# Monokaix/etcd

Hardware: AMD Instinct MI355X
Metric: quorum group-evals/sec at 1/2/4/8 MI355X; % HBM peak; speedup vs Go host (higher is better)
Workload: dtype u64; 1 GPU; config2_n5: 64M groups x 5-voter MajorityConfig CommittedIndex+VoteResult (TallyVotes counts into the stats); groups_per_gpu=67108864, global_groups=67108864, voters=5

## Files before the change

### etcd_amd/csrc/qe_api.hip

```cpp
#include <stdio.h>
#include <string.h>

#include "qe_dispatch.hpp"
#include "qe_conf.hpp"
#include "qe_collect.hpp"
#include "qe_tick.hpp"
#include "qe_follow.hpp"
#include "qe_vote.hpp"
#include "qe_snap.hpp"
#include "qe_outbox.hpp"
#include "qe_inbox.hpp"
#include "qe_replies.hpp"

namespace qe {

int g_blocks_per_cu = 0;
int g_nontemporal = 3;
int g_tiles_per_wave = -1;
int g_cv_kernel = -1;
int g_repl_kernel = -1;

static thread_local char g_errbuf[256];

void set_error(const char *msg) { snprintf(g_errbuf, sizeof(g_errbuf), "%s", msg); }

int hip_status(hipError_t e) {
  if (e == hipSuccess) return QE_OK;
  snprintf(g_errbuf, sizeof(g_errbuf), "HIP error %d: %s", static_cast<int>(e),
           hipGetErrorString(e));
  return QE_EHIP;
}

static inline bool al(const void *p, size_t a) {
  return (reinterpret_cast<uintptr_t>(p) % a) == 0;
}

static unsigned simple_grid(uint64_t G) {
  const uint64_t cap = static_cast<uint64_t>(num_cus()) * 8;
  const uint64_t need = (G + kBlock - 1) / kBlock;
  return static_cast<unsigned>(need < cap ? (need ? need : 1) : cap);
}

__global__ __launch_bounds__(kBlock) void k_apply_acks(uint64_t G, uint32_t S, uint64_t stride,
                                                       uint64_t *match, uint64_t *next,
                                                       uint64_t n, const uint64_t *group,
                                                       const int8_t *slot,
                                                       const uint64_t *index,
                                                       uint8_t *touched) {
  for (uint64_t i = static_cast<uint64_t>(blockIdx.x) * kBlock + threadIdx.x; i < n;
       i += static_cast<uint64_t>(gridDim.x) * kBlock) {
    const uint64_t g = group[i];
    const int s = slot[i];
    if (g >= G || s < 0 || s >= static_cast<int>(S)) continue;
    const uint64_t x = index[i];
    const uint64_t off = static_cast<uint64_t>(s) * stride + g;
    atomicMax(reinterpret_cast<unsigned long long *>(match + off),
              static_cast<unsigned long long>(x));
    if (x != ~0ull)
      atomicMax(reinterpret_cast<unsigned long long *>(next + off),
                static_cast<unsigned long long>(x + 1));
    if (touched) touched[g] = 1;
  }
}

__global__ void k_stats_reduce(const uint64_t *stats, uint64_t *out) {
  const int c = threadIdx.x;
  if (c < QE_STATS_COUNTERS) {
    uint64_t s = 0;
    for (int k = 0; k < QE_STATS_SHARDS; k++) s += stats[k * QE_STATS_COUNTERS + c];
    out[c] = s;
  }
}


}

using namespace qe;

template <class A>
static void step_head(const qe_progress *p, uint64_t *stats, A &a) {
  a.G = p->num_groups;
  a.goff = p->group_offset;
  a.stride = p->stride;
  a.R = p->log_runs;
  a.stats = stats;
}

extern "C" {

int qe_abi_version(void) { return QE_ABI_VERSION; }

const char *qe_strerror(int status) {
  switch (status) {
    case QE_OK: return "ok";
    case QE_EINVAL: return "invalid argument";
    case QE_ERANGE: return "out of range";
    case QE_EHIP: return g_errbuf[0] ? g_errbuf : "HIP error";
    case QE_ECOMM: return g_errbuf[0] ? g_errbuf : "RCCL error";
    default: return "unknown status";
  }
}

size_t qe_mask_bytes(uint32_t num_slots) {
  if (num_slots == 0 || num_slots > QE_MAX_SLOTS) return 0;
  return num_slots <= 8 ? 1 : 2;
}

int qe_tune(const char *key, int value) {
  if (!key) return QE_EINVAL;
  if (!strcmp(key, "blocks_per_cu")) {
    if (value < 0 || value > 32) return QE_ERANGE;
    g_blocks_per_cu = value;
    return QE_OK;
  }
  if (!strcmp(key, "tiles_per_wave")) {
    if (value < -1 || value > 4096) return QE_ERANGE;
    g_tiles_per_wave = value;
    return QE_OK;
  }
  if (!strcmp(key, "cv_kernel")) {
    if (value < -1 || value > 1) return QE_ERANGE;
    g_cv_kernel = value;
    return QE_OK;
  }
  if (!strcmp(key, "repl_kernel")) {
    if (value < -1 || value > 1) return QE_ERANGE;
    g_repl_kernel = value;
    return QE_OK;
  }
  if (!strcmp(key, "nontemporal")) {
    if (value < 0 || value > 3) return QE_ERANGE;
    g_nontemporal = value;
    return QE_OK;
  }
  return QE_EINVAL;
}

static int check_groups(const qe_groups *g) {
  if (!g) return QE_EINVAL;
  if (g->num_slots == 0 || g->num_slots > QE_MAX_SLOTS) return QE_EINVAL;
  if (g->reserved != 0) return QE_EINVAL;
  if (g->num_groups && g->stride < g->num_groups) return QE_EINVAL;
  if (g->out_mask && !g->inc_mask) return QE_EINVAL;
  return QE_OK;
}

int qe_commit_vote(const qe_groups *g, const qe_outputs *out, void *stream) {
  int rc = check_groups(g);
  if (rc) return rc;
  if (!out) return QE_EINVAL;
  if (g->num_groups == 0) return QE_OK;
  if (!g->match) return QE_EINVAL;
  CVArgs a{};
  a.G = g->num_groups;
  a.goff = g->group_offset;
  a.stride = g->stride;
  a.match = g->match;
  a.inc = g->inc_mask;
  a.out = g->out_mask;
  a.learner = g->learner_mask;
  a.voted = g->voted;
  a.granted = g->granted;
  a.commit = out->commit;
  a.vote = out->vote;
  a.gcount = out->granted_count;
  a.rcount = out->rejected_count;
  a.stats = out->stats;
  const int mode = g->out_mask ? 2 : (g->inc_mask ? 1 : 0);
  const size_t mb = qe_mask_bytes(g->num_slots);
  bool vec = al(g->match, 16) && (g->stride % 2 == 0) && al(out->commit, 16);
  const void *masks[] = {g->inc_mask, g->out_mask, g->learner_mask, g->voted, g->granted};
  for (const void *m : masks) vec = vec && al(m, 2 * mb);
  const uint8_t *bytes[] = {out->vote, out->granted_count, out->rejected_count};
  for (const uint8_t *b : bytes) vec = vec && al(b, 2);
  return with_slots(g->num_slots, [&](auto s) {
    return dispatch_cv<s()>(a, mode, vec, static_cast<hipStream_t>(stream));
  });
}

int qe_committed_index(const qe_groups *g, uint64_t *commit, void *stream) {
  if (!g || !commit) return QE_EINVAL;
  qe_groups gg = *g;
  gg.voted = nullptr;
  gg.granted = nullptr;
  qe_outputs o{};
  o.commit = commit;
  return qe_commit_vote(&gg, &o, stream);
}

int qe_vote_result(const qe_groups *g, uint8_t *vote, void *stream) {
  int rc = check_groups(g);
  if (rc) return rc;
  if (!vote) return QE_EINVAL;
  if (g->num_groups == 0) return QE_OK;
  const uint32_t full = (1u << g->num_slots) - 1u;
  hipStream_t st = static_cast<hipStream_t>(stream);
  const unsigned grid = simple_grid(g->num_groups);
  if (g->num_slots <= 8)
    hipLaunchKernelGGL(k_vote_result<uint8_t>, dim3(grid), dim3(kBlock), 0, st, g->num_groups,
                       full, g->inc_mask, g->out_mask, g->voted, g->granted, vote);
  else
    hipLaunchKernelGGL(k_vote_result<uint16_t>, dim3(grid), dim3(kBlock), 0, st,
                       g->num_groups, full, g->inc_mask, g->out_mask, g->voted, g->granted,
                       vote);
  return hip_status(hipGetLastError());
}

int qe_quorum_active(const qe_groups *g, const void *recent_active, uint8_t *active,
                     void *stream) {
  int rc = check_groups(g);
  if (rc) return rc;
  if (!recent_active || !active) return QE_EINVAL;
  if (g->num_groups == 0) return QE_OK;
  const uint32_t full = (1u << g->num_slots) - 1u;
  hipStream_t st = static_cast<hipStream_t>(stream);
  const unsigned grid = simple_grid(g->num_groups);
  if (g->num_slots <= 8)
    hipLaunchKernelGGL(k_quorum_active<uint8_t>, dim3(grid), dim3(kBlock), 0, st,
                       g->num_groups, full, g->inc_mask, g->out_mask, g->learner_mask,
                       recent_active, active);
  else
    hipLaunchKernelGGL(k_quorum_active<uint16_t>, dim3(grid), dim3(kBlock), 0, st,
                       g->num_groups, full, g->inc_mask, g->out_mask, g->learner_mask,
                       recent_active, active);
  return hip_status(hipGetLastError());
}

int qe_record_votes(uint64_t num_groups, uint32_t num_slots, void *voted, void *granted,
                    const void *resp_mask, const void *resp_value, void *stream) {
  if (num_slots == 0 || num_slots > QE_MAX_SLOTS) return QE_EINVAL;
  if (num_groups == 0) return QE_OK;
  if (!voted || !granted || !resp_mask || !resp_value) return QE_EINVAL;
  const uint32_t full = (1u << num_slots) - 1u;
  hipStream_t st = static_cast<hipStream_t>(stream);
  const unsigned grid = simple_grid(num_groups);
  if (num_slots <= 8)
    hipLaunchKernelGGL(k_record_votes<uint8_t>, dim3(grid), dim3(kBlock), 0, st, num_groups,
                       full, voted, granted, resp_mask, resp_value);
  else
    hipLaunchKernelGGL(k_record_votes<uint16_t>, dim3(grid), dim3(kBlock), 0, st, num_groups,
                       full, voted, granted, resp_mask, resp_value);
  return hip_status(hipGetLastError());
}

int qe_replication_round(const qe_repl_state *s, const qe_repl_msgs *m, uint64_t *stats,
                         void *stream) {
  if (!s || !m) return QE_EINVAL;
  if (s->num_slots == 0 || s->num_slots > QE_MAX_SLOTS || s->reserved) return QE_EINVAL;
  if (s->num_groups == 0) return QE_OK;
  if (s->stride < s->num_groups) return QE_EINVAL;
  if (!s->match || !s->next || !s->committed || !s->term_start || !s->last_index ||
      !m->resp_index)
    return QE_EINVAL;
  if (s->out_mask && !s->inc_mask) return QE_EINVAL;
  RArgs a{};
  a.G = s->num_groups;
  a.goff = s->group_offset;
  a.stride = s->stride;
  a.match = s->match;
  a.next = s->next;
  a.committed = s->committed;
  a.term_start = s->term_start;
  a.last_index = s->last_index;
  a.resp = m->resp_index;
  a.inc = s->inc_mask;
  a.out = s->out_mask;
  a.resp_mask = m->resp_mask;
  a.read_acks = m->read_acks;
  a.read_ok = m->read_ok;
  a.adv = m->commit_advanced;
  a.stats = stats;
  const size_t mb = qe_mask_bytes(s->num_slots);
  bool vec = (s->stride % 2 == 0);
  const void *p16[] = {s->match, s->next, s->committed, s->term_start, s->last_index,
                       m->resp_index};
// ... 940 lines not shown
```

### etcd_amd/csrc/qe_inst.hip

```cpp
#include "qe_dispatch.hpp"

#ifndef QE_S
#error "compile with -DQE_S=<slots>"
#endif
#ifndef QE_PAIRS
#define QE_PAIRS ((QE_S) <= 8 ? 2 : 1)
#endif

namespace qe {

namespace {
constexpr int S = QE_S;
using MT = std::conditional<(S <= 8), uint8_t, uint16_t>::type;

template <int MODE, bool VEC, bool NTL, bool NTS>
int launch_cv_k(const CVArgs &a, hipStream_t st) {
  constexpr int kPairs = QE_PAIRS;
  auto kern = k_commit_vote<S, MODE, MT, kPairs, VEC, NTL, NTS>;
  static int occ = occupancy(kern);
  const uint64_t npairs = (a.G + 1) / 2;
  const uint64_t tiles = (npairs + 64 * kPairs - 1) / (64 * kPairs);
  hipLaunchKernelGGL(kern, dim3(grid_for(tiles, occ, MODE == 2 ? 8 : 1)), dim3(kBlock), 0, st, a);
  return hip_status(hipGetLastError());
}

ChunkPlan stream_plan(uint64_t G) {
  return chunk_plan((G + 63) / 64, num_cus(), g_tiles_per_wave, QE_STREAM_TPW, false);
}

template <int MODE, bool NTL, bool NTS>
int launch_cv_stream(CVArgs a, hipStream_t st) {
  auto kern = k_cv_stream<S, MODE, MT, NTL, NTS>;
  const ChunkPlan plan = stream_plan(a.G);
  if (plan.status) return plan.status;
  a.chunk = plan.chunk;
  hipLaunchKernelGGL(kern, dim3(plan.blocks), dim3(kBlock), 0, st, a);
  return hip_status(hipGetLastError());
}

template <int MODE>
int launch_cv(const CVArgs &a, bool vec, hipStream_t st) {
  const int which = g_cv_kernel >= 0 ? g_cv_kernel : 1;
  if (which == 1)
    return with_nontemporal(g_nontemporal, [&](auto ntl, auto nts) {
      return launch_cv_stream<MODE, ntl(), nts()>(a, st);
    });
  if (!vec) return launch_cv_k<MODE, false, false, false>(a, st);
  return with_nontemporal(g_nontemporal, [&](auto ntl, auto nts) {
    return launch_cv_k<MODE, true, ntl(), nts()>(a, st);
  });
}
}

template <int N>
int dispatch_cv(const CVArgs &a, int mode, bool vec, hipStream_t st) {
  static_assert(N == S, "one slot count per object");
  switch (mode) {
    case 0: return launch_cv<0>(a, vec, st);
    case 1: return launch_cv<1>(a, vec, st);
    default: return launch_cv<2>(a, vec, st);
  }
}
template int dispatch_cv<S>(const CVArgs &, int, bool, hipStream_t);

template <bool J, bool M, bool V, bool NT>
static int launch_repl_k(const RArgs &a, hipStream_t st) {
  auto kern = k_replication<S, J, M, MT, V, NT>;
  static int occ = occupancy(kern);
  const uint64_t tiles = ((a.G + 1) / 2 + 63) / 64;
  hipLaunchKernelGGL(kern, dim3(grid_for(tiles, occ, 1)), dim3(kBlock), 0, st, a);
  return hip_status(hipGetLastError());
}

template <bool J, bool M, bool V>
static int launch_repl(const RArgs &a, hipStream_t st) {
  if (V && (g_nontemporal & 3) == 3) return launch_repl_k<J, M, V, true>(a, st);
  return launch_repl_k<J, M, V, false>(a, st);
}

template <bool M, bool J, bool NTL, bool NTS>
static int launch_repl_stream(RArgs a, hipStream_t st) {
  auto kern = k_repl_stream<S, M, J, MT, NTL, NTS>;
  const ChunkPlan plan = stream_plan(a.G);
  if (plan.status) return plan.status;
  a.chunk = plan.chunk;
  hipLaunchKernelGGL(kern, dim3(plan.blocks), dim3(kBlock), 0, st, a);
  return hip_status(hipGetLastError());
}

template <int N>
int dispatch_repl(const RArgs &a, bool masked, bool joint, bool vec, hipStream_t st) {
  static_assert(N == S, "one slot count per object");
  if (g_repl_kernel != 0)
    return with_quorum_form(masked, joint, [&](auto m, auto j) {
      return with_nontemporal(g_nontemporal, [&](auto ntl, auto nts) {
        return launch_repl_stream<m(), j(), ntl(), nts()>(a, st);
      });
    });
  if (vec)
    return with_quorum_form(masked, joint,
                            [&](auto m, auto j) { return launch_repl<j(), m(), true>(a, st); });
  return with_quorum_form(masked, joint,
                          [&](auto m, auto j) { return launch_repl<j(), m(), false>(a, st); });
}
template int dispatch_repl<S>(const RArgs &, bool, bool, bool, hipStream_t);

template <int OPT>
static int launch_elec(const EArgs &a, hipStream_t st) {
  auto kern = k_election<S, MT, OPT>;
  static int occ = occupancy(kern);
  const uint64_t waves = (a.G + 63) / 64;
  hipLaunchKernelGGL(kern, dim3(grid_for(waves, occ, 1)), dim3(kBlock), 0, st, a);
  return hip_status(hipGetLastError());
}

template <int N>
int dispatch_elec(const EArgs &a, hipStream_t st) {
  static_assert(N == S, "one slot count per object");
  const int opt = (a.flags & 3u) | (a.sresp ? 4 : 0) | (a.out ? 8 : 0);
  switch (opt) {
#define QE_E(o) \
  case o: return launch_elec<o>(a, st);
    QE_E(0) QE_E(1) QE_E(2) QE_E(3) QE_E(4) QE_E(5) QE_E(6) QE_E(7)
    QE_E(8) QE_E(9) QE_E(10) QE_E(11) QE_E(12) QE_E(13) QE_E(14)
#undef QE_E
    default: return launch_elec<15>(a, st);
  }
}
template int dispatch_elec<S>(const EArgs &, hipStream_t);

}
```

### etcd_amd/csrc/qe_kernels.hpp

```cpp
#pragma once
#if !defined(QE_VARIANT_BUILD) &&                                                      \
    (defined(QE_PSTEP_WAVES) || defined(QE_STREAM_TPW) || defined(QE_STREAM_WAVES) ||     \
     defined(QE_JOINT_MIN_WAVES) || defined(QE_LD_AUX) || defined(QE_ST_AUX) ||           \
     defined(QE_SEND_AUX) || defined(QE_SEND16_WAVES) || defined(QE_SWITCH16_WAVES) ||    \
     defined(QE_PROPOSE16_WAVES))
#error "A/B knob set in a product build: use scripts/build_variant*.sh (QE_VARIANT_BUILD)"
#endif
#include <hip/hip_runtime.h>

#include <stdint.h>
#include <stdio.h>
#include <string.h>

#include <type_traits>

#include "../../include/etcd_quorum.h"
#include "qe_device.hpp"
#include "qe_launch.hpp"

namespace qe {

typedef uint64_t u64x2 __attribute__((ext_vector_type(2)));

extern int g_blocks_per_cu;
extern int g_nontemporal;
extern int g_cv_kernel;
extern int g_repl_kernel;

inline int num_cus() {
  static int cached[64] = {0};
  int dev = 0;
  if (hipGetDevice(&dev) != hipSuccess || dev < 0 || dev >= 64) return 256;
  if (cached[dev] == 0) {
    int v = 0;
    if (hipDeviceGetAttribute(&v, hipDeviceAttributeMultiprocessorCount, dev) != hipSuccess ||
        v <= 0)
      v = 256;
    cached[dev] = v;
  }
  return cached[dev];
}

extern int g_tiles_per_wave;
inline unsigned grid_for(uint64_t work_waves, int occ, int auto_tpw = 0) {
  const uint64_t need = (work_waves + (kBlock / 64) - 1) / (kBlock / 64);
  const int tpw = g_tiles_per_wave >= 0 ? g_tiles_per_wave : auto_tpw;
  uint64_t g;
  if (tpw > 0) {
    g = (need + tpw - 1) / tpw;
  } else {
    int per_cu = occ > 0 ? occ : 4;
    if (g_blocks_per_cu > 0 && g_blocks_per_cu < per_cu) per_cu = g_blocks_per_cu;
    const uint64_t cap = static_cast<uint64_t>(num_cus()) * per_cu;
    g = need < cap ? need : cap;
  }
  if (g > 0x7FFFFFFFull) g = 0x7FFFFFFFull;
  return static_cast<unsigned>(g ? g : 1);
}

template <typename K>
inline int occupancy(K kernel) {
  int n = 0;
  if (hipOccupancyMaxActiveBlocksPerMultiprocessor(&n, kernel, kBlock, 0) != hipSuccess) n = 0;
  return n;
}

template <bool VEC, bool NT, bool GUARD = true>
__device__ __forceinline__ void ld_u64_pair(const uint64_t *p, uint64_t g0, uint64_t G,
                                            uint64_t &lo, uint64_t &hi) {
  if (VEC && (!GUARD || g0 + 1 < G)) {
    const u64x2 *q = reinterpret_cast<const u64x2 *>(p + g0);
    u64x2 x = NT ? __builtin_nontemporal_load(q) : *q;
    lo = x.x;
    hi = x.y;
  } else {
    lo = g0 < G ? p[g0] : 0;
    hi = g0 + 1 < G ? p[g0 + 1] : 0;
  }
}

template <bool VEC, bool NT = false, bool GUARD = true>
__device__ __forceinline__ void st_u64_pair(uint64_t *p, uint64_t g0, uint64_t G, uint64_t lo,
                                            uint64_t hi) {
  if (VEC && (!GUARD || g0 + 1 < G)) {
    u64x2 x;
    x.x = lo;
    x.y = hi;
    if (NT) __builtin_nontemporal_store(x, reinterpret_cast<u64x2 *>(p + g0));
    else *reinterpret_cast<u64x2 *>(p + g0) = x;
  } else {
    if (g0 < G) p[g0] = lo;
    if (g0 + 1 < G) p[g0 + 1] = hi;
  }
}

template <typename MT, bool VEC, bool GUARD = true>
__device__ __forceinline__ void ld_mask_pair(const void *p, uint64_t g0, uint64_t G,
                                             uint32_t &lo, uint32_t &hi) {
  const MT *m = static_cast<const MT *>(p);
  if (VEC && (!GUARD || g0 + 1 < G)) {
    if constexpr (sizeof(MT) == 1) {
      const uint32_t x = *reinterpret_cast<const uint16_t *>(m + g0);
      lo = x & 0xFFu;
      hi = x >> 8;
    } else {
      const uint32_t x = *reinterpret_cast<const uint32_t *>(m + g0);
      lo = x & 0xFFFFu;
      hi = x >> 16;
    }
  } else {
    lo = g0 < G ? m[g0] : 0u;
    hi = g0 + 1 < G ? m[g0 + 1] : 0u;
  }
}

template <typename MT, bool VEC, bool GUARD = true>
__device__ __forceinline__ void st_mask_pair(void *p, uint64_t g0, uint64_t G, uint32_t lo,
                                             uint32_t hi) {
  MT *m = static_cast<MT *>(p);
  if (VEC && (!GUARD || g0 + 1 < G)) {
    if constexpr (sizeof(MT) == 1) {
      *reinterpret_cast<uint16_t *>(m + g0) = static_cast<uint16_t>(lo | (hi << 8));
    } else {
      *reinterpret_cast<uint32_t *>(m + g0) = lo | (hi << 16);
    }
  } else {
    if (g0 < G) m[g0] = static_cast<MT>(lo);
    if (g0 + 1 < G) m[g0 + 1] = static_cast<MT>(hi);
  }
}

template <bool VEC, bool NT = false, bool GUARD = true>
__device__ __forceinline__ void st_u8_pair(uint8_t *p, uint64_t g0, uint64_t G, uint32_t lo,
                                           uint32_t hi) {
  if (VEC && (!GUARD || g0 + 1 < G)) {
    const uint16_t x = static_cast<uint16_t>(lo | (hi << 8));
    if (NT) __builtin_nontemporal_store(x, reinterpret_cast<uint16_t *>(p + g0));
    else *reinterpret_cast<uint16_t *>(p + g0) = x;
  } else {
    if (g0 < G) p[g0] = static_cast<uint8_t>(lo);
    if (g0 + 1 < G) p[g0 + 1] = static_cast<uint8_t>(hi);
  }
}

struct CVArgs {
  uint64_t G, goff, stride;
  const uint64_t *match;
  const void *inc, *out, *learner, *voted, *granted;
  uint64_t *commit;
  uint8_t *vote, *gcount, *rcount;
  uint64_t *stats;
  uint32_t chunk;
};

enum { C_GROUPS, C_INF, C_SUM, C_ZERO, C_WON, C_LOST, C_PEND, C_GR, C_RJ, C_VIOL, C_CSUM, C_N };

template <int S, int MODE>
__device__ __forceinline__ void eval_group(uint64_t (&v)[S], uint32_t inc, uint32_t out,
                                           uint32_t learner, uint32_t voted, uint32_t granted,
                                           uint64_t &commit, uint32_t &vote, uint32_t &gc,
                                           uint32_t &rc, uint32_t top = S) {
  constexpr uint32_t kFull = (1u << S) - 1u;
  if constexpr (MODE == 0) {
    commit = select_fixed<S>(v);
    inc = kFull;
    out = 0;
  } else {
    if constexpr (MODE == 1) out = 0;
    commit = joint_committed_top<S>(v, inc, out, top);
  }
  vote = joint_vote(inc, out, voted, granted);
  const uint32_t voters = (inc | out) & ~learner;
  gc = popc(voted & granted & voters);
  rc = popc(voted & ~granted & voters);
}

struct CVStats {
  uint32_t groups = 0, inf = 0, zero = 0, won = 0, lost = 0, pend = 0, gr = 0, rj = 0, viol = 0;
  uint64_t sum = 0, csum = 0;
};

template <typename MT, int MODE, int PAIRS, bool VEC, bool GUARD>
__device__ __forceinline__ void cv_masks(const CVArgs &a, uint64_t t, int lane,
                                         uint32_t (&mi)[PAIRS][2], uint32_t (&mo)[PAIRS][2]) {
  constexpr uint64_t kTile = 64ull * PAIRS;
#pragma unroll
  for (int j = 0; j < PAIRS; j++) {
    const uint64_t g0 = 2 * (t * kTile + j * 64 + lane);
    ld_mask_pair<MT, VEC, GUARD>(a.inc, g0, a.G, mi[j][0], mi[j][1]);
    if constexpr (MODE == 2) ld_mask_pair<MT, VEC, GUARD>(a.out, g0, a.G, mo[j][0], mo[j][1]);
    else mo[j][0] = mo[j][1] = 0;
  }
}

template <int S, int MODE, typename MT, int PAIRS, bool VEC, bool NTL, bool NTS, bool GUARD>
__device__ __forceinline__ void cv_tile(const CVArgs &a, uint64_t t, int lane, bool want_stats,
                                        CVStats &st, const uint32_t (&mi_in)[PAIRS][2],
                                        const uint32_t (&mo_in)[PAIRS][2], uint64_t tn,
                                        uint64_t ntiles, uint64_t nfull,
                                        uint32_t (&mi_n)[PAIRS][2], uint32_t (&mo_n)[PAIRS][2]) {
  constexpr uint32_t kFull = (1u << S) - 1u;
  constexpr uint64_t kTile = 64ull * PAIRS;
  const uint64_t G = a.G;
  uint64_t v[PAIRS][2][S];
  uint32_t mi[PAIRS][2], mo[PAIRS][2], ml[PAIRS][2], vd[PAIRS][2], gr[PAIRS][2];
  uint32_t used = kFull;
  if constexpr (MODE >= 1) {
    uint32_t u = 0;
#pragma unroll
    for (int j = 0; j < PAIRS; j++)
#pragma unroll
      for (int h = 0; h < 2; h++) {
        mi[j][h] = mi_in[j][h];
        mo[j][h] = mo_in[j][h];
        u |= mi[j][h] | mo[j][h];
      }
    used = wave_or(u) & kFull;
  } else {
#pragma unroll
    for (int j = 0; j < PAIRS; j++) {
      mi[j][0] = mi[j][1] = kFull;
      mo[j][0] = mo[j][1] = 0;
    }
  }
#pragma unroll
  for (int j = 0; j < PAIRS; j++) {
    const uint64_t g0 = 2 * (t * kTile + j * 64 + lane);
#pragma unroll
    for (int s = 0; s < S; s++) {
      if (MODE == 0 || ((used >> s) & 1u))
        ld_u64_pair<VEC, NTL, GUARD>(a.match + s * a.stride, g0, G, v[j][0][s], v[j][1][s]);
      else
        v[j][0][s] = v[j][1][s] = 0;
    }
    if (a.learner) ld_mask_pair<MT, VEC, GUARD>(a.learner, g0, G, ml[j][0], ml[j][1]);
    else ml[j][0] = ml[j][1] = 0;
    if (a.voted) {
      ld_mask_pair<MT, VEC, GUARD>(a.voted, g0, G, vd[j][0], vd[j][1]);
      if (a.granted) ld_mask_pair<MT, VEC, GUARD>(a.granted, g0, G, gr[j][0], gr[j][1]);
      else gr[j][0] = gr[j][1] = 0;
    } else {
      vd[j][0] = vd[j][1] = gr[j][0] = gr[j][1] = 0;
    }
  }
  if constexpr (MODE >= 1) {
    if (tn < ntiles) {
      if (VEC && tn < nfull) cv_masks<MT, MODE, PAIRS, VEC, false>(a, tn, lane, mi_n, mo_n);
      else cv_masks<MT, MODE, PAIRS, VEC, true>(a, tn, lane, mi_n, mo_n);
    }
  }
#pragma unroll
  for (int j = 0; j < PAIRS; j++) {
    const uint64_t g0 = 2 * (t * kTile + j * 64 + lane);
    uint64_t c[2];
    uint32_t vt[2], gc[2], rc[2];
#pragma unroll
    for (int h = 0; h < 2; h++) {
      const uint32_t inc = mi[j][h] & kFull, out = mo[j][h] & kFull, lrn = ml[j][h] & kFull;
      const uint32_t vv = vd[j][h] & kFull, gg = gr[j][h] & kFull;
      eval_group<S, MODE>(v[j][h], inc, out, lrn, vv, gg, c[h], vt[h], gc[h], rc[h]);
      if (want_stats && (!GUARD || g0 + h < G)) {
        st.groups += 1;
        st.inf += (c[h] == kInf);
        st.sum += (c[h] == kInf) ? 0 : c[h];
        st.zero += (c[h] == 0);
        st.won += (vt[h] == kVoteWon);
        st.lost += (vt[h] == kVoteLost);
        st.pend += (vt[h] == kVotePending);
        st.gr += gc[h];
        st.rj += rc[h];
        st.viol += ((lrn & (inc | out)) != 0);
        const uint64_t tag = static_cast<uint64_t>(vt[h] | (gc[h] << 2) | (rc[h] << 7)) << 52;
        st.csum += mix64(((a.goff + g0 + h) * kPhi) ^ c[h] ^ tag);
      }
    }
    if (a.commit) st_u64_pair<VEC, NTS, GUARD>(a.commit, g0, G, c[0], c[1]);
    if (a.vote) st_u8_pair<VEC, NTS, GUARD>(a.vote, g0, G, vt[0], vt[1]);
    if (a.gcount) st_u8_pair<VEC, NTS, GUARD>(a.gcount, g0, G, gc[0], gc[1]);
    if (a.rcount) st_u8_pair<VEC, NTS, GUARD>(a.rcount, g0, G, rc[0], rc[1]);
  }
}

#ifndef QE_JOINT_MIN_WAVES
#define QE_JOINT_MIN_WAVES 1
#endif
template <int S, int MODE, typename MT, int PAIRS, bool VEC, bool NTL, bool NTS>
__global__ __attribute__((amdgpu_flat_work_group_size(1, kBlock),
                          amdgpu_waves_per_eu(MODE == 2 ? QE_JOINT_MIN_WAVES : 1)))
void k_commit_vote(CVArgs a) {
  const int lane = threadIdx.x & 63;
  const uint64_t wave = (static_cast<uint64_t>(blockIdx.x) * kBlock + threadIdx.x) >> 6;
  const uint64_t nwaves = (static_cast<uint64_t>(gridDim.x) * kBlock) >> 6;
  const uint64_t npairs = (a.G + 1) >> 1;
  constexpr uint64_t kTile = 64ull * PAIRS;
  const uint64_t ntiles = (npairs + kTile - 1) / kTile;
  const uint64_t nfull = a.G / (2 * kTile);
  const bool want_stats = a.stats != nullptr;

  CVStats st;
  uint32_t mi[PAIRS][2] = {}, mo[PAIRS][2] = {};
  if constexpr (MODE >= 1) {
    if (wave < ntiles) {
      if (VEC && wave < nfull) cv_masks<MT, MODE, PAIRS, VEC, false>(a, wave, lane, mi, mo);
      else cv_masks<MT, MODE, PAIRS, VEC, true>(a, wave, lane, mi, mo);
    }
// ... 584 lines not shown
```

### etcd_amd/csrc/qe_launch.hpp

```cpp
#pragma once
#include <stdint.h>

#include <type_traits>

#include "../../include/etcd_quorum.h"

namespace qe {

constexpr int kBlock = 256;

struct ChunkPlan {
  int status;
  uint32_t chunk, blocks;
};

inline ChunkPlan chunk_plan(uint64_t tiles, int cus, int tpw_override, uint32_t max_tpw,
                            bool floor_override) {
  uint64_t chunk;
  if (tpw_override > 0) {
    chunk = static_cast<uint64_t>(tpw_override);
    if (floor_override && chunk < 2) chunk = 2;
  } else {
    const uint64_t waves = static_cast<uint64_t>(cus) * 32;
    chunk = (tiles + waves - 1) / waves;
    if (chunk < 2) chunk = 2;
  }
  if (chunk > max_tpw) chunk = max_tpw;
  const uint64_t per_block = (kBlock / 64) * chunk;
  const uint64_t blocks = (tiles + per_block - 1) / per_block;
  if (blocks > 0x7FFFFFFFull) return {QE_ERANGE, 0, 0};
  return {QE_OK, static_cast<uint32_t>(chunk), static_cast<uint32_t>(blocks)};
}

inline uint32_t tile_grid(uint64_t groups, int cus, bool stats) {
  const uint64_t tiles = (groups + 63) / 64;
  uint64_t blocks = (tiles + (kBlock / 64) - 1) / (kBlock / 64);
  const uint64_t cap = stats ? static_cast<uint64_t>(cus) * 8 : 0x7FFFFFFFull;
  if (blocks > cap) blocks = cap;
  return static_cast<uint32_t>(blocks ? blocks : 1);
}

template <class F>
inline int with_quorum_form(bool masked, bool joint, F &&f) {
  if (joint) return f(std::true_type{}, std::true_type{});
  if (masked) return f(std::true_type{}, std::false_type{});
  return f(std::false_type{}, std::false_type{});
}

template <class F>
inline int with_nontemporal(int bits, F &&f) {
  switch (bits & 3) {
    case 1: return f(std::true_type{}, std::false_type{});
    case 2: return f(std::false_type{}, std::true_type{});
    case 3: return f(std::true_type{}, std::true_type{});
    default: return f(std::false_type{}, std::false_type{});
  }
}

template <int N>
using slots_c = std::integral_constant<int, N>;

template <class F>
inline int with_slots(uint32_t S, F &&f) {
  static_assert(QE_MAX_SLOTS == 16, "one case per slot count");
  switch (S) {
    case 1: return f(slots_c<1>{});
    case 2: return f(slots_c<2>{});
    case 3: return f(slots_c<3>{});
    case 4: return f(slots_c<4>{});
    case 5: return f(slots_c<5>{});
    case 6: return f(slots_c<6>{});
    case 7: return f(slots_c<7>{});
    case 8: return f(slots_c<8>{});
    case 9: return f(slots_c<9>{});
    case 10: return f(slots_c<10>{});
    case 11: return f(slots_c<11>{});
    case 12: return f(slots_c<12>{});
    case 13: return f(slots_c<13>{});
    case 14: return f(slots_c<14>{});
    case 15: return f(slots_c<15>{});
    case 16: return f(slots_c<16>{});
    default: return QE_EINVAL;
  }
}

}
```

### etcd_amd/csrc/qe_stream.hpp

```cpp
#pragma once
#include "qe_kernels.hpp"

namespace qe {

typedef __amdgpu_buffer_rsrc_t rsrc_t;
constexpr uint32_t kOOB = 0x80000000u;

__device__ __forceinline__ uint32_t bit_off(uint32_t mask, int s, uint32_t off) {
  return ((~mask << (31 - s)) & kOOB) | off;
}

__device__ __forceinline__ rsrc_t mk_rsrc(const void *p, uint32_t bytes) {
  return __builtin_amdgcn_make_buffer_rsrc(const_cast<void *>(p), 0, static_cast<int>(bytes),
                                           0x00020000);
}

template <typename MT>
__device__ __forceinline__ uint32_t bld_mask(const void *base, uint64_t tile0, uint32_t n,
                                             uint32_t lane) {
  const rsrc_t r = mk_rsrc(static_cast<const MT *>(base) + tile0, n * sizeof(MT));
  if constexpr (sizeof(MT) == 1)
    return __builtin_amdgcn_raw_buffer_load_b8(r, lane, 0, 0);
  else
    return __builtin_amdgcn_raw_buffer_load_b16(r, lane * 2, 0, 0);
}

struct STile {
  uint32_t lrn, vd, gr;
};

__device__ __forceinline__ uint32_t tile_n(uint64_t G, uint64_t t) {
  const uint64_t tile0 = t * 64;
  const uint64_t rem = G > tile0 ? G - tile0 : 0;
  return rem < 64 ? static_cast<uint32_t>(rem) : 64u;
}

template <typename T>
__device__ __forceinline__ rsrc_t opt_rsrc(const T *p, uint64_t tile0, uint32_t n) {
  return p ? mk_rsrc(p + tile0, n * sizeof(T)) : mk_rsrc(p, 0);
}

template <typename MT>
__device__ __forceinline__ uint32_t ld_mask_r(rsrc_t r, uint32_t lane) {
  if constexpr (sizeof(MT) == 1)
    return __builtin_amdgcn_raw_buffer_load_b8(r, lane, 0, 0);
  else
    return __builtin_amdgcn_raw_buffer_load_b16(r, lane * 2, 0, 0);
}

template <int S, int MODE, typename MT, bool NTL>
__device__ __forceinline__ void st_issue(const CVArgs &a, uint64_t t, uint32_t lane, uint32_t use,
                                         uint32_t top, uint64_t (&v)[S], STile &x) {
  const uint64_t tile0 = t * 64;
  const uint32_t n = tile_n(a.G, t);
  const uint32_t off = lane * 8;
#pragma unroll
  for (int s = 0; s < S; s++) {
    const rsrc_t r = mk_rsrc(a.match + s * a.stride + tile0, n * 8);
    const uint32_t o = MODE == 0 ? off : bit_off(use, s, off);
    if (MODE != 0 && static_cast<uint32_t>(s) >= top) {
      v[s] = 0;
      continue;
    }
    v[s] = __builtin_bit_cast(uint64_t, __builtin_amdgcn_raw_buffer_load_b64(r, o, 0, NTL ? 2 : 0));
  }
  const MT *lp = static_cast<const MT *>(a.learner), *vp = static_cast<const MT *>(a.voted);
  const MT *gp = a.voted ? static_cast<const MT *>(a.granted) : nullptr;
  x.lrn = ld_mask_r<MT>(opt_rsrc(lp, tile0, n), lane);
  x.vd = ld_mask_r<MT>(opt_rsrc(vp, tile0, n), lane);
  x.gr = ld_mask_r<MT>(opt_rsrc(gp, tile0, n), lane);
}

template <int S, int MODE, bool NTS>
__device__ __forceinline__ void st_finish(const CVArgs &a, uint64_t t, uint32_t lane,
                                          bool want_stats, uint32_t mio, uint32_t top,
                                          uint64_t (&v)[S], const STile &x, CVStats &st) {
  constexpr uint32_t kFull = (1u << S) - 1u;
  const uint64_t tile0 = t * 64;
  const uint32_t n = tile_n(a.G, t);
  const uint32_t inc = MODE == 0 ? kFull : (mio & kFull);
  const uint32_t out = MODE == 2 ? ((mio >> 16) & kFull) : 0u;
  const uint32_t lrn = x.lrn & kFull, vv = x.vd & kFull, gg = x.gr & kFull;
  uint64_t c;
  uint32_t vt, gc, rc;
  eval_group<S, MODE>(v, inc, out, lrn, vv, gg, c, vt, gc, rc, top);
  if (want_stats && lane < n) {
    st.groups += 1;
    st.inf += (c == kInf);
    st.sum += (c == kInf) ? 0 : c;
    st.zero += (c == 0);
    st.won += (vt == kVoteWon);
    st.lost += (vt == kVoteLost);
    st.pend += (vt == kVotePending);
    st.gr += gc;
    st.rj += rc;
    st.viol += ((lrn & (inc | out)) != 0);
    const uint64_t tag = static_cast<uint64_t>(vt | (gc << 2) | (rc << 7)) << 52;
    st.csum += mix64(((a.goff + tile0 + lane) * kPhi) ^ c ^ tag);
  }
  const int aux = NTS ? 2 : 0;
  typedef uint32_t u32x2 __attribute__((ext_vector_type(2)));
  __builtin_amdgcn_raw_buffer_store_b64(__builtin_bit_cast(u32x2, c), opt_rsrc(a.commit, tile0, n),
                                        lane * 8, 0, aux);
  __builtin_amdgcn_raw_buffer_store_b8(static_cast<uint8_t>(vt), opt_rsrc(a.vote, tile0, n), lane,
                                       0, aux);
  __builtin_amdgcn_raw_buffer_store_b8(static_cast<uint8_t>(gc), opt_rsrc(a.gcount, tile0, n),
                                       lane, 0, aux);
  __builtin_amdgcn_raw_buffer_store_b8(static_cast<uint8_t>(rc), opt_rsrc(a.rcount, tile0, n),
                                       lane, 0, aux);
}

#ifndef QE_STREAM_TPW
#define QE_STREAM_TPW 8
#endif

#ifndef QE_STREAM_WAVES
#define QE_STREAM_WAVES 1
#endif

template <int S, int MODE, typename MT, bool NTL, bool NTS>
__global__ __attribute__((amdgpu_flat_work_group_size(1, kBlock),
                          amdgpu_waves_per_eu(QE_STREAM_WAVES))) void k_cv_stream(CVArgs a) {
  constexpr int TPW = QE_STREAM_TPW;
  __shared__ uint32_t lds_m[kBlock / 64][TPW][64];
  const uint32_t lane = threadIdx.x & 63;
  const uint32_t w = __builtin_amdgcn_readfirstlane(threadIdx.x >> 6);
  const uint64_t ntiles = (a.G + 63) / 64;
  const uint32_t chunk = a.chunk;
  const uint64_t t0 = (static_cast<uint64_t>(blockIdx.x) * (kBlock / 64) + w) * chunk;
  const uint32_t nt =
      t0 < ntiles ? static_cast<uint32_t>(ntiles - t0 < chunk ? ntiles - t0 : chunk) : 0u;
  const bool want_stats = a.stats != nullptr;
  CVStats st;
  uint32_t top = S;
  if (nt > 0) {
    if constexpr (MODE >= 1) {
      uint32_t mv[TPW];
#pragma unroll
      for (int k = 0; k < TPW; k++) {
        const uint64_t tile0 = (t0 + k) * 64;
        const uint32_t n = tile_n(a.G, t0 + k);
        uint32_t m = bld_mask<MT>(a.inc, tile0, n, lane);
        if constexpr (MODE == 2) m |= bld_mask<MT>(a.out, tile0, n, lane) << 16;
        mv[k] = m;
      }
      uint32_t any = 0;
#pragma unroll
      for (int k = 0; k < TPW; k++) {
        lds_m[w][k][lane] = mv[k];
        any |= mv[k];
      }
      top = __builtin_amdgcn_readfirstlane(
          32u - __builtin_clz(wave_or((any | (any >> 16)) & 0xFFFFu) | 1u));
    }
    auto use_of = [&](uint32_t k) -> uint32_t {
      if constexpr (MODE == 0) return 0u;
      const uint32_t m = lds_m[w][k][lane];
      return MODE == 2 ? ((m | (m >> 16)) & 0xFFFFu) : m;
    };
    auto mio_of = [&](uint32_t k) -> uint32_t {
      if constexpr (MODE == 0) return 0u;
      return lds_m[w][k][lane];
    };
    const uint64_t tend = t0 + nt;
    auto tix = [&](uint32_t k) -> uint64_t { return t0 + k < tend ? t0 + k : ntiles; };
    uint64_t va[S], vb[S];
    STile xa, xb;
    st_issue<S, MODE, MT, NTL>(a, tix(0), lane, use_of(0), top, va, xa);
    for (uint32_t k = 0; k < nt; k += 2) {
      st_issue<S, MODE, MT, NTL>(a, tix(k + 1), lane, use_of((k + 1) % TPW), top, vb, xb);
      __builtin_amdgcn_sched_barrier(0);
      st_finish<S, MODE, NTS>(a, tix(k), lane, want_stats, mio_of(k), top, va, xa, st);
      st_issue<S, MODE, MT, NTL>(a, tix(k + 2), lane, use_of((k + 2) % TPW), top, va, xa);
      __builtin_amdgcn_sched_barrier(0);
      st_finish<S, MODE, NTS>(a, tix(k + 1), lane, want_stats, mio_of((k + 1) % TPW), top, vb,
                              xb, st);
    }
  }
  if (want_stats) {
    uint64_t cnt[C_N] = {st.groups, st.inf, st.sum, st.zero, st.won, st.lost,
                         st.pend,   st.gr,  st.rj,  st.viol, st.csum};
    const int idx[C_N] = {QE_STAT_GROUPS,     QE_STAT_COMMIT_INF,   QE_STAT_COMMIT_SUM,
                          QE_STAT_COMMIT_ZERO, QE_STAT_VOTE_WON,    QE_STAT_VOTE_LOST,
                          QE_STAT_VOTE_PENDING, QE_STAT_GRANTED,    QE_STAT_REJECTED,
                          QE_STAT_INVARIANT_VIOLATIONS, QE_STAT_CHECKSUM};
    block_stats_add<C_N, kBlock>(cnt, idx, a.stats);
  }
}

}
```

Before: 122.3 billion group-evals/s.

## Add wide-row chunk path to streaming commit/vote kernel with LDS byte staging

Adds a wide path for full 8-tile chunks. Each lane loads 8 consecutive mask bytes (64/128-bit loads) for the inc/out/learner/voted/granted arrays and stages them through LDS, instead of issuing per-tile byte loads. The vote/gcount/rcount byte outputs are gathered in LDS and written as 64-bit stores, replacing per-lane byte stores. Per-slot waves_per_eu hints are also tuned from a table. The aim is fewer, wider memory transactions for the byte arrays, at the cost of extra LDS use, alignment checks and a second code path.

```diff
diff --git a/etcd_amd/csrc/qe_api.hip b/etcd_amd/csrc/qe_api.hip
--- a/etcd_amd/csrc/qe_api.hip
+++ b/etcd_amd/csrc/qe_api.hip
@@ -19,6 +19,7 @@
 int g_tiles_per_wave = -1;
 int g_cv_kernel = -1;
 int g_repl_kernel = -1;
+int g_cv_wide = -1;
 
 static thread_local char g_errbuf[256];
 
@@ -121,6 +122,11 @@
   if (!strcmp(key, "cv_kernel")) {
     if (value < -1 || value > 1) return QE_ERANGE;
     g_cv_kernel = value;
+    return QE_OK;
+  }
+  if (!strcmp(key, "cv_wide")) {
+    if (value < -1 || value > 1) return QE_ERANGE;
+    g_cv_wide = value;
     return QE_OK;
   }
   if (!strcmp(key, "repl_kernel")) {
diff --git a/etcd_amd/csrc/qe_inst.hip b/etcd_amd/csrc/qe_inst.hip
--- a/etcd_amd/csrc/qe_inst.hip
+++ b/etcd_amd/csrc/qe_inst.hip
@@ -34,6 +34,9 @@
   const ChunkPlan plan = stream_plan(a.G);
   if (plan.status) return plan.status;
   a.chunk = plan.chunk;
+  a.wide = g_cv_wide != 0 && QE_STREAM_TPW == kWideTiles && a.commit != nullptr &&
+           wide_rows_ok(plan.chunk, sizeof(MT), {a.inc, a.out, a.learner, a.voted, a.granted},
+                        {a.vote, a.gcount, a.rcount});
   hipLaunchKernelGGL(kern, dim3(plan.blocks), dim3(kBlock), 0, st, a);
   return hip_status(hipGetLastError());
 }
diff --git a/etcd_amd/csrc/qe_kernels.hpp b/etcd_amd/csrc/qe_kernels.hpp
--- a/etcd_amd/csrc/qe_kernels.hpp
+++ b/etcd_amd/csrc/qe_kernels.hpp
@@ -26,6 +26,7 @@
 extern int g_nontemporal;
 extern int g_cv_kernel;
 extern int g_repl_kernel;
+extern int g_cv_wide;
 
 inline int num_cus() {
   static int cached[64] = {0};
@@ -151,6 +152,7 @@
   uint8_t *vote, *gcount, *rcount;
   uint64_t *stats;
   uint32_t chunk;
+  uint32_t wide;
 };
 
 enum { C_GROUPS, C_INF, C_SUM, C_ZERO, C_WON, C_LOST, C_PEND, C_GR, C_RJ, C_VIOL, C_CSUM, C_N };
diff --git a/etcd_amd/csrc/qe_launch.hpp b/etcd_amd/csrc/qe_launch.hpp
--- a/etcd_amd/csrc/qe_launch.hpp
+++ b/etcd_amd/csrc/qe_launch.hpp
@@ -1,6 +1,8 @@
 #pragma once
+#include <stddef.h>
 #include <stdint.h>
 
+#include <initializer_list>
 #include <type_traits>
 
 #include "../../include/etcd_quorum.h"
@@ -30,6 +32,23 @@
   const uint64_t blocks = (tiles + per_block - 1) / per_block;
   if (blocks > 0x7FFFFFFFull) return {QE_ERANGE, 0, 0};
   return {QE_OK, static_cast<uint32_t>(chunk), static_cast<uint32_t>(blocks)};
+}
+
+constexpr uint32_t kWideTiles = 8;
+
+inline bool wide_rows_ok(uint32_t chunk, size_t mask_bytes,
+                         std::initializer_list<const void *> masks,
+                         std::initializer_list<const void *> bytes) {
+  if (chunk != kWideTiles) return false;
+  for (const void *p : masks)
+    if (p && reinterpret_cast<uintptr_t>(p) % (8 * mask_bytes) != 0) return false;
+  for (const void *p : bytes)
+    if (p && reinterpret_cast<uintptr_t>(p) % 8 != 0) return false;
+  return true;
+}
+
+constexpr bool wide_chunk_ok(uint64_t G, uint64_t t0, uint32_t nt) {
+  return nt == kWideTiles && (t0 + kWideTiles) * 64 <= G;
 }
 
 inline uint32_t tile_grid(uint64_t groups, int cus, bool stats) {
diff --git a/etcd_amd/csrc/qe_stream.hpp b/etcd_amd/csrc/qe_stream.hpp
--- a/etcd_amd/csrc/qe_stream.hpp
+++ b/etcd_amd/csrc/qe_stream.hpp
@@ -48,11 +48,10 @@
     return __builtin_amdgcn_raw_buffer_load_b16(r, lane * 2, 0, 0);
 }
 
-template <int S, int MODE, typename MT, bool NTL>
-__device__ __forceinline__ void st_issue(const CVArgs &a, uint64_t t, uint32_t lane, uint32_t use,
-                                         uint32_t top, uint64_t (&v)[S], STile &x) {
+template <int S, int MODE, bool NTL>
+__device__ __forceinline__ void st_rows(const CVArgs &a, uint64_t t, uint32_t n, uint32_t lane,
+                                        uint32_t use, uint32_t top, uint64_t (&v)[S]) {
   const uint64_t tile0 = t * 64;
-  const uint32_t n = tile_n(a.G, t);
   const uint32_t off = lane * 8;
 #pragma unroll
   for (int s = 0; s < S; s++) {
@@ -64,25 +63,30 @@
     }
     v[s] = __builtin_bit_cast(uint64_t, __builtin_amdgcn_raw_buffer_load_b64(r, o, 0, NTL ? 2 : 0));
   }
+}
+
+template <typename MT>
+__device__ __forceinline__ void st_bytes(const CVArgs &a, uint64_t t, uint32_t n, uint32_t lane,
+                                         STile &x) {
+  const uint64_t tile0 = t * 64;
   const MT *lp = static_cast<const MT *>(a.learner), *vp = static_cast<const MT *>(a.voted);
   const MT *gp = a.voted ? static_cast<const MT *>(a.granted) : nullptr;
-  x.lrn = ld_mask_r<MT>(opt_rsrc(lp, tile0, n), lane);
-  x.vd = ld_mask_r<MT>(opt_rsrc(vp, tile0, n), lane);
-  x.gr = ld_mask_r<MT>(opt_rsrc(gp, tile0, n), lane);
-}
-
-template <int S, int MODE, bool NTS>
-__device__ __forceinline__ void st_finish(const CVArgs &a, uint64_t t, uint32_t lane,
-                                          bool want_stats, uint32_t mio, uint32_t top,
-                                          uint64_t (&v)[S], const STile &x, CVStats &st) {
+  x.lrn = x.vd = x.gr = 0;
+  if (lp) x.lrn = ld_mask_r<MT>(mk_rsrc(lp + tile0, n * sizeof(MT)), lane);
+  if (vp) x.vd = ld_mask_r<MT>(mk_rsrc(vp + tile0, n * sizeof(MT)), lane);
+  if (gp) x.gr = ld_mask_r<MT>(mk_rsrc(gp + tile0, n * sizeof(MT)), lane);
+}
+
+template <int S, int MODE>
+__device__ __forceinline__ void st_eval(const CVArgs &a, uint64_t t, uint32_t n, uint32_t lane,
+                                        bool want_stats, uint32_t mio, uint32_t top,
+                                        uint64_t (&v)[S], const STile &x, CVStats &st, uint64_t &c,
+                                        uint32_t &vt, uint32_t &gc, uint32_t &rc) {
   constexpr uint32_t kFull = (1u << S) - 1u;
   const uint64_t tile0 = t * 64;
-  const uint32_t n = tile_n(a.G, t);
   const uint32_t inc = MODE == 0 ? kFull : (mio & kFull);
   const uint32_t out = MODE == 2 ? ((mio >> 16) & kFull) : 0u;
   const uint32_t lrn = x.lrn & kFull, vv = x.vd & kFull, gg = x.gr & kFull;
-  uint64_t c;
-  uint32_t vt, gc, rc;
   eval_group<S, MODE>(v, inc, out, lrn, vv, gg, c, vt, gc, rc, top);
   if (want_stats && lane < n) {
     st.groups += 1;
@@ -98,16 +102,28 @@
     const uint64_t tag = static_cast<uint64_t>(vt | (gc << 2) | (rc << 7)) << 52;
     st.csum += mix64(((a.goff + tile0 + lane) * kPhi) ^ c ^ tag);
   }
+}
+
+typedef uint32_t u32x2 __attribute__((ext_vector_type(2)));
+typedef uint32_t u32x4 __attribute__((ext_vector_type(4)));
+
+template <bool NTS>
+__device__ __forceinline__ void st_store(const CVArgs &a, uint64_t t, uint32_t n, uint32_t lane,
+                                         uint64_t c, uint32_t vt, uint32_t gc, uint32_t rc) {
+  const uint64_t tile0 = t * 64;
   const int aux = NTS ? 2 : 0;
-  typedef uint32_t u32x2 __attribute__((ext_vector_type(2)));
-  __builtin_amdgcn_raw_buffer_store_b64(__builtin_bit_cast(u32x2, c), opt_rsrc(a.commit, tile0, n),
-                                        lane * 8, 0, aux);
-  __builtin_amdgcn_raw_buffer_store_b8(static_cast<uint8_t>(vt), opt_rsrc(a.vote, tile0, n), lane,
-                                       0, aux);
-  __builtin_amdgcn_raw_buffer_store_b8(static_cast<uint8_t>(gc), opt_rsrc(a.gcount, tile0, n),
-                                       lane, 0, aux);
-  __builtin_amdgcn_raw_buffer_store_b8(static_cast<uint8_t>(rc), opt_rsrc(a.rcount, tile0, n),
-                                       lane, 0, aux);
+  if (a.commit)
+    __builtin_amdgcn_raw_buffer_store_b64(__builtin_bit_cast(u32x2, c),
+                                          mk_rsrc(a.commit + tile0, n * 8), lane * 8, 0, aux);
+  if (a.vote)
+    __builtin_amdgcn_raw_buffer_store_b8(static_cast<uint8_t>(vt), mk_rsrc(a.vote + tile0, n),
+                                         lane, 0, aux);
+  if (a.gcount)
+    __builtin_amdgcn_raw_buffer_store_b8(static_cast<uint8_t>(gc), mk_rsrc(a.gcount + tile0, n),
+                                         lane, 0, aux);
+  if (a.rcount)
+    __builtin_amdgcn_raw_buffer_store_b8(static_cast<uint8_t>(rc), mk_rsrc(a.rcount + tile0, n),
+                                         lane, 0, aux);
 }
 
 #ifndef QE_STREAM_TPW
@@ -118,11 +134,191 @@
 #define QE_STREAM_WAVES 1
 #endif
 
+constexpr int kWideGroups = static_cast<int>(kWideTiles) * 64;
+enum { W_LRN, W_VD, W_GR, W_IN };
+enum { W_VOTE, W_GC, W_RC, W_OUT };
+
+template <typename MT>
+struct alignas(16) WideLds {
+  MT in[W_IN][kWideGroups];
+};
+
+template <typename MT>
+using wide_t = typename std::conditional<sizeof(MT) == 1, u32x2, u32x4>::type;
+typedef u32x2 __attribute__((may_alias)) u32x2_lds;
+typedef u32x4 __attribute__((may_alias)) u32x4_lds;
+typedef uint16_t __attribute__((may_alias)) u16_lds;
+
+__device__ __forceinline__ void wave_fence() {
+  __builtin_amdgcn_fence(__ATOMIC_ACQ_REL, "wavefront");
+}
+
+template <typename MT, bool NT>
+__device__ __forceinline__ wide_t<MT> wide_ld(const void *base, uint64_t g0, uint32_t lane) {
+  const rsrc_t r = mk_rsrc(static_cast<const MT *>(base) + g0, kWideGroups * sizeof(MT));
+  if constexpr (sizeof(MT) == 1)
+    return __builtin_bit_cast(u32x2,
+                              __builtin_amdgcn_raw_buffer_load_b64(r, lane * 8, 0, NT ? 2 : 0));
+  else
+    return __builtin_bit_cast(u32x4,
+                              __builtin_amdgcn_raw_buffer_load_b128(r, lane * 16, 0, NT ? 2 : 0));
+}
+
+template <typename MT>
+__device__ __forceinline__ uint32_t wide_at(wide_t<MT> v, int j) {
+  if constexpr (sizeof(MT) == 1)
+    return (v[j >> 2] >> (8 * (j & 3))) & 0xFFu;
+  else
+    return (v[j >> 1] >> (16 * (j & 1))) & 0xFFFFu;
+}
+
+template <typename MT>
+__device__ __forceinline__ uint32_t wide_any(wide_t<MT> v) {
+  if constexpr (sizeof(MT) == 1) {
+    const uint32_t x = v[0] | v[1];
+    return (x | (x >> 8) | (x >> 16) | (x >> 24)) & 0xFFu;
+  } else {
+    const uint32_t x = v[0] | v[1] | v[2] | v[3];
+    return (x | (x >> 16)) & 0xFFFFu;
+  }
+}
+
+template <typename MT>
+__device__ __forceinline__ void wide_stage(MT (&row)[kWideGroups], wide_t<MT> v, uint32_t lane) {
+  if constexpr (sizeof(MT) == 1)
+    *reinterpret_cast<u32x2_lds *>(&row[lane * 8]) = v;
+  else
+    *reinterpret_cast<u32x4_lds *>(&row[lane * 8]) = v;
+}
+
+template <typename MT>
+__device__ __forceinline__ uint32_t wide_get(const MT (&row)[kWideGroups], uint32_t k,
+                                             uint32_t lane) {
+  if constexpr (sizeof(MT) == 1)
+    return row[k * 64 + lane];
+  else
+    return *reinterpret_cast<const u16_lds *>(&row[k * 64 + lane]);
+}
+
+template <int S, int MODE, typename MT, bool NTL, bool NTS>
+__device__ __forceinline__ void cv_chunk_wide(const CVArgs &a, uint64_t t0, uint32_t lane,
+                                              bool want_stats, uint32_t (&lm)[QE_STREAM_TPW][64],
+                                              WideLds<MT> &wl, CVStats &st) {
+  constexpr int TPW = static_cast<int>(kWideTiles);
+  static_assert(QE_STREAM_TPW >= TPW, "the voter-mask image holds the chunk");
+  const uint64_t g0 = t0 * 64;
+  const void *gp = a.voted ? a.granted : nullptr;
+  wide_t<MT> bl = {}, bv = {}, bg = {};
+  if (a.learner) bl = wide_ld<MT, NTL>(a.learner, g0, lane);
+  if (a.voted) bv = wide_ld<MT, NTL>(a.voted, g0, lane);
+  if (gp) bg = wide_ld<MT, NTL>(gp, g0, lane);
+  uint32_t top = S;
+  if constexpr (MODE >= 1) {
+    const wide_t<MT> bi = wide_ld<MT, NTL>(a.inc, g0, lane);
+    wide_t<MT> bo = {};
+    if constexpr (MODE == 2) bo = wide_ld<MT, NTL>(a.out, g0, lane);
+    uint32_t *dst = &lm[0][0] + lane * 8;
+    u32x4 lo, hi;
+#pragma unroll
+    for (int j = 0; j < 4; j++) {
+      lo[j] = wide_at<MT>(bi, j) | (wide_at<MT>(bo, j) << 16);
+      hi[j] = wide_at<MT>(bi, j + 4) | (wide_at<MT>(bo, j + 4) << 16);
+    }
+    *reinterpret_cast<u32x4_lds *>(dst) = lo;
+    *reinterpret_cast<u32x4_lds *>(dst + 4) = hi;
+    top = __builtin_amdgcn_readfirstlane(
+        32u - __builtin_clz(wave_or(wide_any<MT>(bi) | wide_any<MT>(bo)) | 1u));
+    wave_fence();
+  }
+  auto use_of = [&](uint32_t k) -> uint32_t {
+    if constexpr (MODE == 0) return 0u;
+    const uint32_t m = lm[k][lane];
+    return MODE == 2 ? ((m | (m >> 16)) & 0xFFFFu) : m;
+  };
+  auto mio_of = [&](uint32_t k) -> uint32_t {
+    if constexpr (MODE == 0) return 0u;
+    return lm[k][lane];
+  };
+  auto bytes_of = [&](uint32_t k, STile &x) {
+    x.lrn = x.vd = x.gr = 0;
+    if (a.learner) x.lrn = wide_get<MT>(wl.in[W_LRN], k, lane);
+    if (a.voted) x.vd = wide_get<MT>(wl.in[W_VD], k, lane);
+    if (gp) x.gr = wide_get<MT>(wl.in[W_GR], k, lane);
+  };
+  auto finish = [&](uint32_t k, uint64_t (&v)[S]) {
+    uint64_t c;
+    uint32_t vt, gc, rc;
+    STile x;
+    bytes_of(k, x);
+    st_eval<S, MODE>(a, t0 + k, 64u, lane, want_stats, mio_of(k), top, v, x, st, c, vt, gc, rc);
+    __builtin_amdgcn_raw_buffer_store_b64(__builtin_bit_cast(u32x2, c),
+                                          mk_rsrc(a.commit + (t0 + k) * 64, 512), lane * 8, 0,
+                                          NTS ? 2 : 0);
+    lm[k][lane] = vt | (gc << (8 * W_GC)) | (rc << (8 * W_RC));
+  };
+  uint64_t va[S], vb[S];
+  st_rows<S, MODE, NTL>(a, t0, 64u, lane, use_of(0), top, va);
+  if (a.learner) wide_stage<MT>(wl.in[W_LRN], bl, lane);
+  if (a.voted) wide_stage<MT>(wl.in[W_VD], bv, lane);
+  if (gp) wide_stage<MT>(wl.in[W_GR], bg, lane);
+  wave_fence();
+  constexpr uint32_t kT = TPW;
+  constexpr int kSteps = MODE == 0 ? TPW / 2 : 1;
+#pragma unroll kSteps
+  for (uint32_t k = 0; k < kT; k += 2) {
+    st_rows<S, MODE, NTL>(a, t0 + k + 1, 64u, lane, use_of(k + 1), top, vb);
+    __builtin_amdgcn_sched_barrier(0);
+    finish(k, va);
+    if constexpr (MODE == 0) {
+      if (k + 2 < kT) st_rows<S, MODE, NTL>(a, t0 + k + 2, 64u, lane, 0u, top, va);
+    } else {
+      st_rows<S, MODE, NTL>(a, t0 + k + 2, k + 2 < kT ? 64u : 0u, lane,
+                            use_of(k + 2 < kT ? k + 2 : k + 1), top, va);
+    }
+    __builtin_amdgcn_sched_barrier(0);
+    finish(k + 1, vb);
+  }
+  wave_fence();
+  const uint32_t *img = &lm[0][0] + lane * 8;
+  const u32x4 wlo = *reinterpret_cast<const u32x4_lds *>(img);
+  const u32x4 whi = *reinterpret_cast<const u32x4_lds *>(img + 4);
+  uint8_t *const outs[W_OUT] = {a.vote, a.gcount, a.rcount};
+#pragma unroll
+  for (int r = 0; r < W_OUT; r++)
+    if (outs[r]) {
+      u32x2 b = {0, 0};
+#pragma unroll
+      for (int j = 0; j < 4; j++) {
+        b[0] |= ((wlo[j] >> (8 * r)) & 0xFFu) << (8 * j);
+        b[1] |= ((whi[j] >> (8 * r)) & 0xFFu) << (8 * j);
+      }
+      __builtin_amdgcn_raw_buffer_store_b64(b, mk_rsrc(outs[r] + g0, kWideGroups), lane * 8, 0,
+                                            NTS ? 2 : 0);
+    }
+}
+
+template <int S, int MODE>
+constexpr bool stream_wide_built() {
+  if (MODE >= 1) return S != 16;
+  return S != 8 && S != 11 && S != 15;
+}
+
+template <int S, int MODE>
+constexpr int stream_waves() {
+  constexpr int kWaves[3][QE_MAX_SLOTS] = {
+      {8, 8, 8, 8, 8, 8, 8, 8, 7, 6, 6, 5, 5, 5, 5, 4},
+      {8, 8, 8, 8, 7, 5, 4, 4, 4, 4, 4, 3, 3, 3, 3, 3},
+      {8, 8, 8, 7, 6, 4, 4, 4, 4, 4, 3, 3, 3, 3, 3, 3}};
+  if (QE_STREAM_WAVES > 1 || !stream_wide_built<S, MODE>()) return QE_STREAM_WAVES;
+  return kWaves[MODE][S - 1];
+}
+
 template <int S, int MODE, typename MT, bool NTL, bool NTS>
 __global__ __attribute__((amdgpu_flat_work_group_size(1, kBlock),
-                          amdgpu_waves_per_eu(QE_STREAM_WAVES))) void k_cv_stream(CVArgs a) {
+                          amdgpu_waves_per_eu(stream_waves<S, MODE>()))) void k_cv_stream(CVArgs a) {
   constexpr int TPW = QE_STREAM_TPW;
-  __shared__ uint32_t lds_m[kBlock / 64][TPW][64];
+  __shared__ __attribute__((aligned(16))) uint32_t lds_m[kBlock / 64][TPW][64];
+  __shared__ WideLds<MT> lds_w[kBlock / 64];
   const uint32_t lane = threadIdx.x & 63;
   const uint32_t w = __builtin_amdgcn_readfirstlane(threadIdx.x >> 6);
   const uint64_t ntiles = (a.G + 63) / 64;
@@ -133,7 +329,9 @@
   const bool want_stats = a.stats != nullptr;
   CVStats st;
   uint32_t top = S;
-  if (nt > 0) {
+  if (stream_wide_built<S, MODE>() && a.wide && wide_chunk_ok(a.G, t0, nt)) {
+    cv_chunk_wide<S, MODE, MT, NTL, NTS>(a, t0, lane, want_stats, lds_m[w], lds_w[w], st);
+  } else if (nt > 0) {
     if constexpr (MODE >= 1) {
       uint32_t mv[TPW];
 #pragma unroll
@@ -164,17 +362,30 @@
     };
     const uint64_t tend = t0 + nt;
     auto tix = [&](uint32_t k) -> uint64_t { return t0 + k < tend ? t0 + k : ntiles; };
+    auto issue = [&](uint32_t k, uint64_t (&v)[S], STile &x) {
+      const uint64_t t = tix(k);
+      const uint32_t n = tile_n(a.G, t);
+      st_rows<S, MODE, NTL>(a, t, n, lane, use_of(k % TPW), top, v);
+      st_bytes<MT>(a, t, n, lane, x);
+    };
+    auto finish = [&](uint32_t k, uint64_t (&v)[S], const STile &x) {
+      const uint64_t t = tix(k);
+      const uint32_t n = tile_n(a.G, t);
+      uint64_t c;
+      uint32_t vt, gc, rc;
+      st_eval<S, MODE>(a, t, n, lane, want_stats, mio_of(k % TPW), top, v, x, st, c, vt, gc, rc);
+      st_store<NTS>(a, t, n, lane, c, vt, gc, rc);
+    };
     uint64_t va[S], vb[S];
     STile xa, xb;
-    st_issue<S, MODE, MT, NTL>(a, tix(0), lane, use_of(0), top, va, xa);
+    issue(0, va, xa);
     for (uint32_t k = 0; k < nt; k += 2) {
-      st_issue<S, MODE, MT, NTL>(a, tix(k + 1), lane, use_of((k + 1) % TPW), top, vb, xb);
+      issue(k + 1, vb, xb);
       __builtin_amdgcn_sched_barrier(0);
-      st_finish<S, MODE, NTS>(a, tix(k), lane, want_stats, mio_of(k), top, va, xa, st);
-      st_issue<S, MODE, MT, NTL>(a, tix(k + 2), lane, use_of((k + 2) % TPW), top, va, xa);
+      finish(k, va, xa);
+      issue(k + 2, va, xa);
       __builtin_amdgcn_sched_barrier(0);
-      st_finish<S, MODE, NTS>(a, tix(k + 1), lane, want_stats, mio_of((k + 1) % TPW), top, vb,
-                              xb, st);
+      finish(k + 1, vb, xb);
     }
   }
   if (want_stats) {
```

Result: slower. 117.9 billion group-evals/s (-3.7%).
